# 0xSameer/ast

Hardware: AMD Instinct MI355X
Metric: speech frames/s (train step) (higher is better)
Workload: dtype f32 storage / f32 accumulate; batched GEMMs as bf16x3 splits on the bf16 MFMA pipe (every f32 operand value represented EXACTLY by three bf16 terms, f32 exponent range, six term products, each product exact to 2^-26: >= float32 on any data); the encoder recurrences multiply the same way (resident we

## Files before the change

### ast_amd/_lib.py

```python
import ctypes as C
import os

_HERE = os.path.dirname(os.path.abspath(__file__))
LIB_PATH = os.environ.get("ASTK_LIB_PATH") or os.path.join(_HERE, "libastk.so")

TEST_LIB_PATH = os.path.join(_HERE, "libastk_test.so")

MAX_CNN = 4
MAX_RNN = 8
MAX_ATTN = 4
ENCODE_ROWS_MAX = 32
PREC_DEFAULT, PREC_FP16X2, PREC_BF16X3, PREC_F32 = 0, 1, 2, 3
OPERANDS_DEFAULT, OPERANDS_F32, OPERANDS_FP16 = 0, 1, 2
OPERANDS_BY_NAME = {None: OPERANDS_DEFAULT, "default": OPERANDS_DEFAULT, "f32": OPERANDS_F32, "fp16": OPERANDS_FP16}
PREC_BY_NAME = {None: PREC_DEFAULT, "default": PREC_DEFAULT, "fp16x2": PREC_FP16X2, "bf16x3": PREC_BF16X3, "f32": PREC_F32}

c_float_p = C.POINTER(C.c_float)
c_int_p = C.POINTER(C.c_int32)
c_double_p = C.POINTER(C.c_double)


class _Sized:

    def __init__(self, *a, **k):
# ... 178 lines not shown
    "astk_sample_topk_workspace_bytes": (_SZ, [C.POINTER(DecoderDesc), _I]),
    "astk_sample_decode_topk": (C.c_int, [C.POINTER(DecoderDesc), C.POINTER(DecoderParams), _VP, _VP, _VP, _I, _I, _I, _VP, _F, _I, _F, _VP,
                                          _VP, _VP, _VP, _VP, _VP, _SZ, _VP, _VP]),
    "astk_gumbel_rows": (C.c_int, [_VP, _I, _I, _I, _VP, _VP]),
    "astk_sample_row_key": (_U64, [_U64, _U64]),
    "astk_forced_workspace_bytes": (_SZ, [C.POINTER(DecoderDesc), _I, _I]),
    "astk_forced_score": (C.c_int, [C.POINTER(DecoderDesc), C.POINTER(DecoderParams), _VP, _VP, _VP, _VP, _I, _VP, _VP, _VP, _VP, _VP, _VP, _SZ,
                                    _VP]),
    "astk_greedy_decode_rows": (C.c_int, [C.POINTER(DecoderDesc), C.POINTER(DecoderParams), _VP, _VP, _VP, _I, _I, _I, _VP, _VP, _VP, _VP,
                                          _SZ, _VP, _VP]),
    "astk_greedy_decode_scored_rows": (C.c_int, [C.POINTER(DecoderDesc), C.POINTER(DecoderParams), _VP, _VP, _VP, _I, _I, _I, _VP, _I, _VP,
                                                 _VP, _VP, _VP, _VP, _VP, _VP, _SZ, _VP, _VP]),
    "astk_sample_decode_rows": (C.c_int, [C.POINTER(DecoderDesc), C.POINTER(DecoderParams), _VP, _VP, _VP, _I, _I, _I, _VP, _F, _VP, _VP, _VP,
                                          _VP, _VP, _SZ, _VP, _VP]),
    "astk_forced_score_rows": (C.c_int, [C.POINTER(DecoderDesc), C.POINTER(DecoderParams), _VP, _VP, _VP, _VP, _I, _VP, _VP, _VP, _VP, _VP,
                                         _VP, _SZ, _VP, _VP]),
    "astk_beam_workspace_bytes": (_SZ, [C.POINTER(BeamDesc), C.POINTER(DecoderDesc)]),
    "astk_beam_step": (C.c_int, [C.POINTER(BeamDesc), C.POINTER(DecoderDesc), C.POINTER(DecoderParams), _VP, C.POINTER(BeamState), _I, _VP,
                                 _SZ, _VP]),
    "astk_beam_select": (C.c_int, [C.POINTER(BeamDesc), _I, _I, _I, _VP, _VP, _L, _VP, _VP, _VP, C.POINTER(BeamState), _I, _VP]),
    "astk_beam_decode_workspace_bytes": (_SZ, [C.POINTER(DecoderDesc), _I, _I, _I, _I]),
    "astk_beam_decode": (C.c_int, [C.POINTER(DecoderDesc), C.POINTER(DecoderParams), _VP, _VP, _VP, _VP, _I, _I, _I, _I, _I, _VP, _VP, _VP, _VP,
                                   _VP, _VP, _VP, _VP, _VP, _VP, _SZ, _VP]),
    "astk_attn_step_fwd_rows": (C.c_int, [_I, _I, _I, _VP, _VP, _VP, _VP, _VP, _VP, _VP, _SZ, _VP]),
    "astk_spin": (C.c_int, [C.c_uint, _VP, _VP]),
    "astk_softmax_ce_fwd": (C.c_int, [_I, _I, _L, _VP, _VP, _L, _VP, _F, _VP, _VP, _VP]),
    "astk_softmax_ce_fwd_ex": (C.c_int, [_I, _I, _L, _VP, _VP, _L, _VP, _F, _F, _VP, _VP, _VP]),
    "astk_grad_sqnorm": (C.c_int, [_VP, _VP, _F, _SZ, _VP, _VP]),
    "astk_decay_clip_amsgrad_step": (C.c_int, [_VP, _VP, _VP, _VP, _VP, _SZ, _F, _F, _VP, _F, C.c_double, C.c_double, _F, _I, _VP]),
    "astk_decay_clip_sgd_step": (C.c_int, [_VP, _VP, _SZ, _F, _F, _VP, _F, _VP]),
    "astk_grad_sqnorm_scaled": (C.c_int, [_VP, _VP, _F, _F, _SZ, _VP, _VP]),
    "astk_decay_clip_amsgrad_step_scaled": (C.c_int, [_VP, _VP, _VP, _VP, _VP, _SZ, _F, _F, _F, _VP, _F, C.c_double, C.c_double, _F, _I, _VP]),
    "astk_decay_clip_sgd_step_scaled": (C.c_int, [_VP, _VP, _SZ, _F, _F, _F, _VP, _F, _VP]),
    "astk_decay_clip_noise": (C.c_int, [_VP, _VP, _SZ, _F, _F, _F, _VP, _F, _U64, _U64, _VP]),
    "astk_fill_dropout_mask": (C.c_int, [_VP, _SZ, _F, _U64, _U64, _VP]),
    "astk_fill_normal": (C.c_int, [_VP, _SZ, _F, _F, _U64, _U64, _VP]),
    "astk_fill_random": (C.c_int, [C.POINTER(RandSeg), _I, _VP]),
    "astk_fill_random_ex": (C.c_int, [C.POINTER(RandSeg), _I, C.POINTER(C.c_int32), _I, _VP, _VP]),
    "astk_scale_f32": (C.c_int, [_VP, _SZ, _F, _VP]),
    "astk_add_f32": (C.c_int, [_VP, _VP, _SZ, _VP]),
    "astk_bridge_states": (C.c_int, [_VP, _VP, _VP, _VP, C.c_int, C.c_int, C.c_int, C.c_int, C.c_int, C.c_int, _VP]),
    "astk_colsum_add_f32": (C.c_int, [_VP, _VP, _L, _I, _I, _VP]),
    "astk_zero_frames": (C.c_int, [_VP, _I, _I, _I, _VP, C.c_double, _U64, _U64, _VP]),
    "astk_zero_frames_draws": (C.c_int, [_I, _I, _VP, C.c_double, _U64, _U64, _VP, _I, _VP, _VP]),
    "astk_persist_status_snapshot": (C.c_int, [_VP, _VP]),
    "astk_persist_status_merge": (C.c_int, [_VP, _VP]),
    "astk_persist_status": (C.c_int, [C.POINTER(C.c_uint), _I]),
    "astk_device_cu_count": (C.c_int, []),
    "astk_lstm_stack_path": (C.c_int, [C.POINTER(LstmStackDesc)]),
    "astk_lstm_stack_free_cus": (C.c_int, [C.POINTER(LstmStackDesc)]),
    "astk_lstm_stack_side_plan": (C.c_int, [C.POINTER(LstmStackDesc), C.POINTER(C.c_int), C.POINTER(C.c_int), C.POINTER(C.c_int)]),
    "astk_decoder_path": (C.c_int, [C.POINTER(DecoderDesc)]),
    "astk_prof_begin": (C.c_int, []),
    "astk_prof_end": (C.c_int, [C.POINTER(C.c_double)]),
}

TEST_HOOK_SIGNATURES = {
    "astk_debug_set_amax_generation": (C.c_int, [C.c_uint]),
    "astk_conv_debug_preact": (C.c_int, [C.POINTER(CnnDesc), _VP, _SZ, _I, _VP, _VP]),
    "astk_conv_debug_kill_units": (C.c_int, [_VP, _I]),
    "astk_debug_gemm_group": (C.c_int, [_I, _I, c_int_p, c_int_p, c_int_p, C.POINTER(C.c_void_p), C.POINTER(C.c_void_p), C.POINTER(C.c_void_p), _I, _I, _VP]),
    "astk_debug_gemm_plan": (C.c_int, [_I, _I] + [c_int_p] * 7 + [_I] * 6 + [C.c_char_p, _SZ]),
    "astk_debug_rowgemm": (C.c_int, [C.POINTER(DebugRowGemmArgs), c_int_p, _VP]),
    "astk_debug_lstm_cell_fwd": (C.c_int, [C.POINTER(DebugCellFwdArgs), _I, c_int_p, _VP]),
    "astk_debug_lstm_cell_bwd": (C.c_int, [C.POINTER(DebugCellBwdArgs), _I, c_int_p, _VP]),
}

_lib = None
_test_lib = None


class AstkError(RuntimeError):
    pass


def load():
    global _lib
    if _lib is not None:
        return _lib
    try:
        import torch
    except ImportError:
        pass
    if not os.path.exists(LIB_PATH):
        raise AstkError(f"{LIB_PATH} not found: build it with `python -c 'import __graft_entry__ as g; g.build()'` "
                        "(there is no CPU or PyTorch fallback for the compute path)")
    lib = C.CDLL(LIB_PATH)
    _bind(lib, SIGNATURES)
    _lib = lib
    return lib


def _bind(lib, sigs):
    for name, (res, args) in sigs.items():
        fn = getattr(lib, name)
# ... 64 lines not shown
```

### ast_amd/csrc/common.h

```cpp
#pragma once
#include <hip/hip_runtime.h>
#include <stdint.h>
#include <stddef.h>
#include <stdio.h>
#include <string.h>
#include "../../include/astk.h"

namespace astk {

void set_error(const char* fmt, ...);

enum ProfCat { PROF_ATTN_FWD = 0, PROF_ATTN_BWD = 1, PROF_GEMM = 2, PROF_CELL = 3, PROF_DEC_FWD = 4, PROF_DEC_BWD = 5, PROF_NCAT = 6 };
bool prof_enabled();
float* prof_tick_buffer(int which);
void prof_start(int cat, hipStream_t s, double work);
void prof_stop(int cat, hipStream_t s);
void prof_add_bytes(int cat, double bytes);
struct ProfScope {
  int cat; hipStream_t s; bool on;
  ProfScope(int c, hipStream_t st, double work = 0.0) : cat(c), s(st), on(prof_enabled()) { if (on) prof_start(cat, s, work); }
  ~ProfScope() { if (on) prof_stop(cat, s); }
};

#define ASTK_CHECK(cond, ...)            \
// ... 3 lines not shown
      return -1;                         \
    }                                    \
  } while (0)

#define ASTK_CHECK_DESC(d, type)                                                                                                        \
  ASTK_CHECK((d) != nullptr && (d)->struct_size == sizeof(type),                                                                         \
             #type ": null descriptor or struct_size %zu != %zu (zero-initialise the struct, set struct_size = sizeof(" #type "), astk.h)", \
             (d) ? (size_t)(d)->struct_size : (size_t)0, sizeof(type))

#define ASTK_HIP(expr)                                                               \
  do {                                                                               \
    hipError_t e_ = (expr);                                                          \
    if (e_ != hipSuccess) {                                                          \
      astk::set_error("%s failed: %s (%s:%d)", #expr, hipGetErrorString(e_), __FILE__, __LINE__); \
      return -2;                                                                     \
    }                                                                                \
  } while (0)

#define ASTK_LAUNCH_CHECK()                                                          \
  do {                                                                               \
    hipError_t e_ = hipGetLastError();                                               \
    if (e_ != hipSuccess) {                                                          \
      astk::set_error("kernel launch failed: %s (%s:%d)", hipGetErrorString(e_), __FILE__, __LINE__); \
      return -3;                                                                     \
    }                                                                                \
  } while (0)

#define ASTK_TRY(expr)        \
  do {                        \
    int r_ = (expr);          \
    if (r_ != 0) return r_;   \
  } while (0)

enum PersistBit { PERSIST_ENC_FWD = 1, PERSIST_ENC_BWD = 2, PERSIST_DEC_FWD = 4, PERSIST_DEC_BWD = 8 };
struct AbortCtl {
  unsigned* word;
  unsigned* status;
  unsigned limit;
  unsigned bit;
};
AbortCtl abort_ctl(unsigned* word, unsigned bit);
int device_cu_count();
enum TuneKey {
  TUNE_GEMM_TILE, TUNE_GEMM_T256_ABOVE, TUNE_GEMM_GRID, TUNE_GEMM_HYBRID, TUNE_GEMM_CHUNK, TUNE_GEMM_CHUNK_DIV, TUNE_GEMM_LOG, TUNE_GEMM_TICKET,
  TUNE_GEMM_DETERMINISTIC, TUNE_GEMM_FORWARD_PAIRS,
  TUNE_CONV_DIRECT0, TUNE_CONV_SEQ_FWD, TUNE_CONV_SEQ_BWD, TUNE_CONV_SEQ_STATS_BLOCKS, TUNE_CONV_SEQ_APPLY_BLOCKS,
  TUNE_DEC_PERSIST, TUNE_DEC_B6_SPLIT, TUNE_DEC_B6_FUSED, TUNE_DEC_WIDE,
  TUNE_LSTM_PERSIST, TUNE_LSTM_HOIST, TUNE_LSTM_X3, TUNE_LSTM_X4, TUNE_LSTM_ROWS32, TUNE_LSTM_OVERLAP_CHUNK, TUNE_LSTM_SIDE_FWD, TUNE_LSTM_SIDE_BWD, TUNE_LSTM_DUO_SIDE,
  TUNE_ROW_LONGK, TUNE_PERSIST_SPIN_LIMIT, TUNE_COLREDUCE_BLOCKS,
  TUNE_COUNT
};
double tune(TuneKey k);
inline bool tune_on(TuneKey k) { return tune(k) != 0.0; }
__device__ __forceinline__ bool abort_seen(const AbortCtl& ab) {
  return __hip_atomic_load(ab.word, __ATOMIC_RELAXED, __HIP_MEMORY_SCOPE_AGENT) != 0;
}
__device__ __forceinline__ void abort_raise(const AbortCtl& ab) {
  __hip_atomic_store(ab.word, 1u, __ATOMIC_RELAXED, __HIP_MEMORY_SCOPE_AGENT);
  __hip_atomic_fetch_or(ab.status, ab.bit, __ATOMIC_RELAXED, __HIP_MEMORY_SCOPE_AGENT);
}

constexpr int AMAX_SLOT_WORDS = 16;
constexpr int AMAX_PSLOT_STRIDE = 16;
constexpr int AMAX_PSLOT_WORDS = AMAX_SLOT_WORDS * AMAX_PSLOT_STRIDE;
static inline unsigned long long* amax_pslot_handle(unsigned long long* p) { return p ? (unsigned long long*)((uintptr_t)p | 1u) : nullptr; }
static inline __host__ __device__ unsigned long long* amax_shard(const unsigned long long* handle, int i) {
  unsigned long long* base = (unsigned long long*)((uintptr_t)handle & ~(uintptr_t)1);
  return base + (i & (AMAX_SLOT_WORDS - 1)) * (((uintptr_t)handle & 1u) ? AMAX_PSLOT_STRIDE : 1);
}

typedef float f32x4 __attribute__((ext_vector_type(4)));
typedef float f32x16 __attribute__((ext_vector_type(16)));
__device__ __forceinline__ float wave_sum(float v) {
#pragma unroll
  for (int o = 32; o > 0; o >>= 1) v += __shfl_xor(v, o);
  return v;
}

#if defined(__HIPCC__)
typedef _Float16 h16x2 __attribute__((ext_vector_type(2)));
typedef _Float16 h16x8 __attribute__((ext_vector_type(8)));
typedef unsigned u32q __attribute__((ext_vector_type(4)));
// ... 440 lines not shown
```

### ast_amd/csrc/util.hip

```cpp
#include "common.h"
#include <algorithm>
#include <stdarg.h>
#include <vector>
#include <atomic>
#include <mutex>

namespace astk {

static thread_local char g_err[512] = "";

void set_error(const char* fmt, ...) {
  va_list ap;
  va_start(ap, fmt);
  vsnprintf(g_err, sizeof(g_err), fmt, ap);
  va_end(ap);
}
const char* last_error() { return g_err; }

struct ProfState {
  bool on = false;
  std::vector<hipEvent_t> ev[PROF_NCAT];
  double work[PROF_NCAT] = {0, 0, 0, 0, 0, 0};
  double bytes[PROF_NCAT] = {0, 0, 0, 0, 0, 0};
};
static ProfState g_prof;
static float* g_tick = nullptr;
float* prof_tick_buffer(int which) { return (g_prof.on && g_tick) ? g_tick + 512 * which : nullptr; }
bool prof_enabled() { return g_prof.on; }
void prof_add_bytes(int cat, double bytes) { if (g_prof.on) g_prof.bytes[cat] += bytes; }
void prof_start(int cat, hipStream_t s, double work) {
  hipEvent_t e;
  if (hipEventCreate(&e) != hipSuccess) return;
  (void)hipEventRecord(e, s);
// ... 34 lines not shown
struct TuneEntry { TuneKey key; const char* name; double def; };
static constexpr TuneEntry g_tune_table[TUNE_COUNT] = {
    {TUNE_GEMM_TILE, "gemm.tile", 0},
    {TUNE_GEMM_T256_ABOVE, "gemm.t256_above", 2e10},
    {TUNE_GEMM_GRID, "gemm.grid", -1},
    {TUNE_GEMM_HYBRID, "gemm.hybrid", 1},
    {TUNE_GEMM_CHUNK, "gemm.chunk", 1},
    {TUNE_GEMM_CHUNK_DIV, "gemm.chunk_div", 4},
    {TUNE_GEMM_LOG, "gemm.log", 0},
    {TUNE_GEMM_TICKET, "gemm.ticket", 1},
    {TUNE_GEMM_DETERMINISTIC, "gemm.deterministic", 0},
    {TUNE_GEMM_FORWARD_PAIRS, "gemm.forward_pairs", 1},
    {TUNE_CONV_DIRECT0, "conv.direct0", 1},
    {TUNE_CONV_SEQ_FWD, "conv.seq_fwd", 1},
    {TUNE_CONV_SEQ_BWD, "conv.seq_bwd", 1},
    {TUNE_CONV_SEQ_STATS_BLOCKS, "conv.seq_stats_blocks", 1024},
    {TUNE_CONV_SEQ_APPLY_BLOCKS, "conv.seq_apply_blocks", 1024},
    {TUNE_DEC_PERSIST, "dec.persist", 1},
    {TUNE_DEC_B6_SPLIT, "dec.b6_split", 1},
    {TUNE_DEC_B6_FUSED, "dec.b6_fused", 1},
    {TUNE_DEC_WIDE, "dec.wide", 1},
    {TUNE_LSTM_PERSIST, "lstm.persist", 1},
    {TUNE_LSTM_HOIST, "lstm.hoist", 1},
    {TUNE_LSTM_X3, "lstm.x3", 1},
    {TUNE_LSTM_X4, "lstm.x4", 1},
    {TUNE_LSTM_ROWS32, "lstm.rows32", -1},
    {TUNE_LSTM_OVERLAP_CHUNK, "lstm.overlap_chunk", 0},
    {TUNE_LSTM_SIDE_FWD, "lstm.side_fwd", 1},
    {TUNE_LSTM_SIDE_BWD, "lstm.side_bwd", 0},
    {TUNE_LSTM_DUO_SIDE, "lstm.duo_side", 0},
    {TUNE_ROW_LONGK, "row.longk", 2048},
    {TUNE_PERSIST_SPIN_LIMIT, "persist.spin_limit", 0},
    {TUNE_COLREDUCE_BLOCKS, "colreduce.blocks", 256},
};
constexpr bool tune_table_in_order() {
  for (int i = 0; i < TUNE_COUNT; ++i)
    if (g_tune_table[i].key != i) return false;
  return true;
}
static_assert(tune_table_in_order(), "g_tune_table rows must follow enum TuneKey");
static std::atomic<double> g_tune[TUNE_COUNT];
static std::atomic<int> g_tune_init{0};
static void tune_init() {
  if (g_tune_init.load(std::memory_order_acquire)) return;
  static std::mutex mu;
  std::lock_guard<std::mutex> lock(mu);
  if (g_tune_init.load()) return;
  for (int i = 0; i < TUNE_COUNT; ++i) g_tune[i].store(g_tune_table[i].def);
  g_tune_init.store(1, std::memory_order_release);
}
double tune(TuneKey k) { tune_init(); return g_tune[k].load(std::memory_order_relaxed); }
static int tune_find(const char* key) {
  if (!key) return -1;
  for (int i = 0; i < TUNE_COUNT; ++i)
    if (!strcmp(key, g_tune_table[i].name)) return i;
  return -1;
}

int device_cu_count() {
  int dev = 0;
  if (hipGetDevice(&dev) != hipSuccess || dev < 0 || dev >= 16) return 0;
  if (g_cu_count[dev] == 0) {
    int n = 0;
    if (hipDeviceGetAttribute(&n, hipDeviceAttributeMultiprocessorCount, dev) != hipSuccess) return 0;
    g_cu_count[dev] = n;
  }
// ... 256 lines not shown
    const float gi = decayed_grad(gi_raw, gsc, l2, pi) * gs;
    mi += omb1 * (gi - mi);
    vi += omb2 * (gi * gi - vi);
    vh = amsgrad ? fmaxf(vh, vi) : vi;
    pi = pi - lr_t * mi / (sqrtf(vh) + eps);
  };
  const size_t stride = (size_t)gridDim.x * blockDim.x, tid = blockIdx.x * (size_t)blockDim.x + threadIdx.x;
  size_t done = 0;
  if (((((uintptr_t)p) | ((uintptr_t)g) | ((uintptr_t)m) | ((uintptr_t)v) | ((uintptr_t)(amsgrad ? vhat : p))) & 15) == 0) {
    const size_t n4 = n / 4;
    float4* p4 = reinterpret_cast<float4*>(p);
    const float4* g4 = reinterpret_cast<const float4*>(g);
    float4 *m4 = reinterpret_cast<float4*>(m), *v4 = reinterpret_cast<float4*>(v), *h4 = reinterpret_cast<float4*>(vhat);
    for (size_t i = tid; i < n4; i += stride) {
      float4 P = p4[i], M = m4[i], V = v4[i], H = amsgrad ? h4[i] : make_float4(0.f, 0.f, 0.f, 0.f);
      const float4 G = g4[i];
      one(P.x, G.x, M.x, V.x, H.x); one(P.y, G.y, M.y, V.y, H.y); one(P.z, G.z, M.z, V.z, H.z); one(P.w, G.w, M.w, V.w, H.w);
      m4[i] = M; v4[i] = V;
      if (amsgrad) h4[i] = H;
      p4[i] = P;
    }
    done = n4 * 4;
  }
  for (size_t i = done + tid; i < n; i += stride) {
    float pi = p[i], mi = m[i], vi = v[i], vh = amsgrad ? vhat[i] : 0.f;
    one(pi, g[i], mi, vi, vh);
    m[i] = mi;
    v[i] = vi;
    if (amsgrad) vhat[i] = vh;
    p[i] = pi;
  }
}

__global__ void k_decay_clip_noise(float* g, const float* p, size_t n, float gsc, float l2, float clip, const double* sqnorm, float sigma,
                                   uint64_t seed, uint64_t offset) {
  const float norm = (float)sqrt(*sqnorm);
  const float rate = clip / norm;
  const float gs = rate < 1.f ? rate : 1.f;
  const size_t pairs = (n + 1) / 2;
  for (size_t i = blockIdx.x * (size_t)blockDim.x + threadIdx.x; i < pairs; i += (size_t)gridDim.x * blockDim.x) {
    const uint64_t b = mix64(seed ^ mix64(offset + i));
    const float u1 = u01(b), u2 = u01(mix64(b));
    const float r = sqrtf(-2.f * logf(u1));
    float sn, cs;
    sincosf(6.2831853071795864f * u2, &sn, &cs);
    g[2 * i] = decayed_grad(g[2 * i], gsc, l2, p[2 * i]) * gs + sigma * r * cs;
    if (2 * i + 1 < n) g[2 * i + 1] = decayed_grad(g[2 * i + 1], gsc, l2, p[2 * i + 1]) * gs + sigma * r * sn;
  }
}

__global__ void k_sgd(float* p, const float* g, size_t n, float gsc, float l2, float clip, const double* sqnorm, float lr, const unsigned* status) {
  if (status && *status != 0u) return;
  const float norm = (float)sqrt(*sqnorm);
  const float rate = clip / norm;
  const float gs = rate < 1.f ? rate : 1.f;
  for (size_t i = blockIdx.x * (size_t)blockDim.x + threadIdx.x; i < n; i += (size_t)gridDim.x * blockDim.x)
    p[i] -= lr * decayed_grad(g[i], gsc, l2, p[i]) * gs;
}

inline unsigned grid_for(size_t n, int per = 256) {
  size_t b = (n + per - 1) / per;
  if (b < 1) b = 1;
  if (b > 2048) b = 2048;
  return (unsigned)b;
}

// ... 149 lines not shown
extern "C" {

int astk_version(void) { return ASTK_VERSION; }
const char* astk_last_error(void) { return astk::last_error(); }

int astk_grad_sqnorm(const float* g, const float* p, float l2, size_t n, double* sqnorm, void* stream) {
  return astk_grad_sqnorm_scaled(g, p, 1.f, l2, n, sqnorm, stream);
}
int astk_grad_sqnorm_scaled(const float* g, const float* p, float grad_scale, float l2, size_t n, double* sqnorm, void* stream) {
  hipStream_t s = (hipStream_t)stream;
  ASTK_CHECK(g && p && sqnorm, "grad_sqnorm: null pointer");
  ASTK_CHECK(aligned16(g) && aligned16(p), "grad_sqnorm: buffers must be 16-byte aligned");
  hipLaunchKernelGGL(k_sqnorm, dim3(std::min(SQNORM_BLOCKS, grid_for(n / 4 + 1))), dim3(256), 0, s, g, p, grad_scale, l2, n, sqnorm);
  ASTK_LAUNCH_CHECK();
  return 0;
}

int astk_decay_clip_amsgrad_step(float* p, const float* g, float* m, float* v, float* vhat, size_t n, float l2, float clip,
                                 const double* sqnorm, float lr_t, double beta1, double beta2, float eps, int amsgrad,
                                 void* stream) {
  return astk_decay_clip_amsgrad_step_scaled(p, g, m, v, vhat, n, 1.f, l2, clip, sqnorm, lr_t, beta1, beta2, eps, amsgrad, stream);
}
int astk_decay_clip_amsgrad_step_scaled(float* p, const float* g, float* m, float* v, float* vhat, size_t n, float grad_scale, float l2,
                                        float clip, const double* sqnorm, float lr_t, double beta1, double beta2, float eps, int amsgrad,
                                        void* stream) {
  ASTK_CHECK(p && g && m && v && sqnorm && (vhat || !amsgrad), "amsgrad_step: null pointer");
  if (n == 0) return 0;
  const float omb1 = (float)(1.0 - beta1), omb2 = (float)(1.0 - beta2);
  hipLaunchKernelGGL(k_amsgrad, dim3(grid_for(n)), dim3(256), 0, (hipStream_t)stream, p, g, m, v, vhat, n, grad_scale, l2, clip, sqnorm,
                     lr_t, omb1, omb2, eps, amsgrad, (const unsigned*)persist_status_ptr());
  ASTK_LAUNCH_CHECK();
  return 0;
}

int astk_decay_clip_sgd_step(float* p, const float* g, size_t n, float l2, float clip, const double* sqnorm, float lr,
                             void* stream) {
  return astk_decay_clip_sgd_step_scaled(p, g, n, 1.f, l2, clip, sqnorm, lr, stream);
}
int astk_decay_clip_sgd_step_scaled(float* p, const float* g, size_t n, float grad_scale, float l2, float clip, const double* sqnorm,
                                    float lr, void* stream) {
  ASTK_CHECK(p && g && sqnorm, "sgd_step: null pointer");
  if (n == 0) return 0;
  hipLaunchKernelGGL(k_sgd, dim3(grid_for(n)), dim3(256), 0, (hipStream_t)stream, p, g, n, grad_scale, l2, clip, sqnorm, lr,
                     (const unsigned*)persist_status_ptr());
  ASTK_LAUNCH_CHECK();
  return 0;
}

int astk_decay_clip_noise(float* g, const float* p, size_t n, float grad_scale, float l2, float clip, const double* sqnorm, float sigma,
                          uint64_t seed, uint64_t offset, void* stream) {
  ASTK_CHECK(g && p && sqnorm && sigma >= 0.f, "decay_clip_noise: bad arguments");
  if (n == 0) return 0;
  hipLaunchKernelGGL(k_decay_clip_noise, dim3(grid_for((n + 1) / 2)), dim3(256), 0, (hipStream_t)stream, g, p, n, grad_scale, l2, clip, sqnorm,
                     sigma, seed, offset);
  ASTK_LAUNCH_CHECK();
  return 0;
}

int astk_fill_dropout_mask(float* out, size_t n, float ratio, uint64_t seed, uint64_t offset, void* stream) {
  ASTK_CHECK(out && ratio >= 0.f && ratio < 1.f, "fill_dropout_mask: bad arguments");
  if (n == 0) return 0;
  hipLaunchKernelGGL(k_dropout_mask, dim3(grid_for(n)), dim3(256), 0, (hipStream_t)stream, out, n, ratio, 1.f / (1.f - ratio),
                     seed, offset);
  ASTK_LAUNCH_CHECK();
  return 0;
}
// ... 201 lines not shown
```

### ast_amd/optimizers.py

```python
import ctypes as C
import math

import torch

from . import _lib
from ._lib import check


class WeightDecay:
    def __init__(self, rate):
        self.rate = rate


class GradientClipping:
    def __init__(self, threshold):
        self.threshold = threshold


class GradientNoise:

    def __init__(self, eta, seed=0x6E015E):
        self.eta = float(eta)
        self.seed = seed
        self.offset = 0
# ... 13 lines not shown
        return self

    def add_hook(self, hook):
        if isinstance(hook, WeightDecay) and any(isinstance(h, (GradientClipping, GradientNoise)) for h in self.hooks):
            raise NotImplementedError("the fused update implements the reference's order WeightDecay -> GradientClipping -> GradientNoise")
        if isinstance(hook, GradientClipping) and any(isinstance(h, GradientNoise) for h in self.hooks):
            raise NotImplementedError("the fused update implements the reference's order WeightDecay -> GradientClipping -> GradientNoise")
        self.hooks.append(hook)

    def _apply_noise(self, lib, a, l2, clip, s):
        noise = [h for h in self.hooks if isinstance(h, GradientNoise)]
        if not noise:
            return l2, clip, self.grad_scale
        h = noise[0]
        sigma = math.sqrt(h.eta / (1.0 + (self.t - 1)) ** 0.55)
        frozen = getattr(self.target, "_frozen", set())
        for name, shp in a.shapes.items():
            if name.split("/")[0] in frozen:
                continue
            off, n = a.offsets[name], 1
            for d in shp:
                n *= int(d)
            check(lib.astk_decay_clip_noise(C.c_void_p(a.grad.data_ptr() + 4 * off), C.c_void_p(a.data.data_ptr() + 4 * off), n, self.grad_scale,
                                            l2, clip, C.c_void_p(self.sqnorm.data_ptr()), sigma, h.seed, h.offset, s))
            h.offset += (n + 1) // 2
        return 0.0, 3.0e38, 1.0

    def _hook_values(self):
        l2 = sum(h.rate for h in self.hooks if isinstance(h, WeightDecay))
        clips = [h.threshold for h in self.hooks if isinstance(h, GradientClipping)]
        clip = float(clips[0]) if clips else float("inf")
        return float(l2), clip

    def _prepare(self):
        m = self.target
        lib = _lib.load()
        a = m.arena
        if self.sqnorm is None:
            self.sqnorm = torch.zeros(1, dtype=torch.float64, device=a.device)
        self.grad_scale = 1.0
        if self.grad_sync is not None:
            r = self.grad_sync(a)
            if isinstance(r, float):
                self.grad_scale = r
        l2, clip = self._hook_values()
        s = C.c_void_p(torch.cuda.current_stream(a.device).cuda_stream)
        check(lib.astk_grad_sqnorm_scaled(C.c_void_p(a.grad.data_ptr()), C.c_void_p(a.data.data_ptr()), self.grad_scale, l2, a.size,
                                          C.c_void_p(self.sqnorm.data_ptr()), s))
        if clip == float("inf"):
            clip = 3.0e38
        return lib, a, l2, clip, s

    @property
    def last_grad_norm(self):
        return math.sqrt(float(self.sqnorm.item()))


class Adam(_Optimizer):
    def __init__(self, alpha=0.001, beta1=0.9, beta2=0.999, eps=1e-8, amsgrad=False):
        super().__init__()
        self.alpha, self.beta1, self.beta2, self.eps, self.amsgrad = alpha, beta1, beta2, eps, amsgrad
        self.m = self.v = self.vhat = None

    def update(self):
        lib, a, l2, clip, s = self._prepare()
        if self.m is None:
            self.m = torch.zeros_like(a.data)
            self.v = torch.zeros_like(a.data)
            self.vhat = torch.zeros_like(a.data)
        self.t += 1
        lr_t = self.alpha * math.sqrt(1.0 - self.beta2 ** self.t) / (1.0 - self.beta1 ** self.t)
        l2, clip, gscale = self._apply_noise(lib, a, l2, clip, s)
        for off, n in self.target.enabled_ranges():
            def p(t):
                return C.c_void_p(t.data_ptr() + 4 * off)
            check(lib.astk_decay_clip_amsgrad_step_scaled(p(a.data), p(a.grad), p(self.m), p(self.v), p(self.vhat), n, gscale, l2,
                                                          clip, C.c_void_p(self.sqnorm.data_ptr()), lr_t, self.beta1, self.beta2,
                                                          self.eps, 1 if self.amsgrad else 0, s))


class SGD(_Optimizer):
    def __init__(self, lr=0.01):
        super().__init__()
        self.lr = lr

    def update(self):
        lib, a, l2, clip, s = self._prepare()
        self.t += 1
        l2, clip, gscale = self._apply_noise(lib, a, l2, clip, s)
        for off, n in self.target.enabled_ranges():
            check(lib.astk_decay_clip_sgd_step_scaled(C.c_void_p(a.data.data_ptr() + 4 * off), C.c_void_p(a.grad.data_ptr() + 4 * off), n,
                                                      gscale, l2, clip, C.c_void_p(self.sqnorm.data_ptr()), self.lr, s))
```

### include/astk.h

```cpp
#ifndef ASTK_H
#define ASTK_H
#include <stddef.h>
#include <stdint.h>

#ifdef __cplusplus
extern "C" {
#endif

#define ASTK_VERSION 108
#define ASTK_MAX_CNN_LAYERS 4
#define ASTK_MAX_RNN_LAYERS 8
#define ASTK_MAX_ATTN 4

int astk_version(void);
const char* astk_last_error(void);

enum { ASTK_PREC_DEFAULT = 0, ASTK_PREC_FP16X2 = 1, ASTK_PREC_BF16X3 = 2, ASTK_PREC_F32 = 3 };
enum { ASTK_OPERANDS_DEFAULT = 0, ASTK_OPERANDS_F32 = 1, ASTK_OPERANDS_FP16 = 2 };

int astk_gemm_f32(int layout, int M, int N, int K,
                  const float* A, long lda, const float* B, long ldb, float* C, long ldc,
                  const float* bias, int mode, int ksplit, int batch, long sA, long sB, long sC, void* stream);
int astk_gemm_f32_ex(int layout, int M, int N, int K,
                     const float* A, long lda, const float* B, long ldb, float* C, long ldc,
// ... 269 lines not shown
                     int32_t* hist, int32_t* slot_status, double* score, float* c_fin, float* h_fin, float* ht_fin, float* alpha,
                     void* ws, size_t ws_bytes, void* stream);

int astk_attn_step_fwd_rows(int R, int T, int H, const float* enc, const int32_t* row_utt, const int32_t* row_len, const float* q,
                            float* alpha, float* cv, void* ws, size_t ws_bytes, void* stream);

int astk_layernorm_fwd(int rows, int n, const float* x, long ldx, const float* gamma, const float* beta, float eps, float* y, long ldy,
                       void* stream);
int astk_layernorm_bwd(int rows, int n, const float* x, long ldx, const float* gamma, float eps, const float* dy, long lddy, float* dx,
                       long lddx, float* dgamma, float* dbeta, void* stream);
int astk_step_bn_relu_fwd(int T, int B, int C, const float* z, const float* gamma, const float* beta, float* avg_mean, float* avg_var,
                          float eps, float decay, int train, float* out, float* stats, void* stream);
int astk_step_bn_relu_bwd(int T, int B, int C, const float* z, const float* stats, const float* gamma, float eps, const float* out,
                          const float* d_out, float* dz, float* dgamma, float* dbeta, void* stream);

int astk_softmax_ce_fwd(int B, int V, long ld, float* logits_inout, const int32_t* targets, long t_stride,
                        const float* class_weight, float inv_count, float* loss_rows, int32_t* argmax, void* stream);
int astk_softmax_ce_fwd_ex(int B, int V, long ld, float* logits_inout, const int32_t* targets, long t_stride,
                           const float* class_weight, float inv_count, float label_smoothing, float* loss_rows, int32_t* argmax,
                           void* stream);

int astk_grad_sqnorm(const float* g, const float* p, float l2, size_t n, double* sqnorm, void* stream);
int astk_decay_clip_amsgrad_step(float* p, const float* g, float* m, float* v, float* vhat, size_t n,
                                 float l2, float clip, const double* sqnorm, float lr_t, double beta1, double beta2,
                                 float eps, int amsgrad, void* stream);
int astk_decay_clip_sgd_step(float* p, const float* g, size_t n, float l2, float clip, const double* sqnorm,
                             float lr, void* stream);
int astk_grad_sqnorm_scaled(const float* g, const float* p, float grad_scale, float l2, size_t n, double* sqnorm, void* stream);
int astk_decay_clip_amsgrad_step_scaled(float* p, const float* g, float* m, float* v, float* vhat, size_t n, float grad_scale,
                                        float l2, float clip, const double* sqnorm, float lr_t, double beta1, double beta2,
                                        float eps, int amsgrad, void* stream);
int astk_decay_clip_sgd_step_scaled(float* p, const float* g, size_t n, float grad_scale, float l2, float clip,
                                    const double* sqnorm, float lr, void* stream);

int astk_fill_dropout_mask(float* out, size_t n, float ratio, uint64_t seed, uint64_t offset, void* stream);
int astk_decay_clip_noise(float* g, const float* p, size_t n, float grad_scale, float l2, float clip, const double* sqnorm, float sigma,
                          uint64_t seed, uint64_t offset, void* stream);
int astk_fill_normal(float* out, size_t n, float mean, float sigma, uint64_t seed, uint64_t offset, void* stream);
#define ASTK_RAND_SEG_MAX 8
#define ASTK_RAND_DROPOUT 0
#define ASTK_RAND_NORMAL 1
typedef struct {
  float* out;
  size_t n;
  int kind;
  float a, b;
  uint64_t seed, offset;
} astk_rand_seg;
int astk_fill_random(const astk_rand_seg* segs, int n_segs, void* stream);
#define ASTK_RAND_WORDS_MAX 256
int astk_fill_random_ex(const astk_rand_seg* segs, int n_segs, const int32_t* words, int n_words, int32_t* words_dst, void* stream);
int astk_scale_f32(float* x, size_t n, float s, void* stream);
int astk_add_f32(float* dst, const float* src, size_t n, void* stream);
int astk_colsum_add_f32(float* dst, const float* src, long lds, int rows, int cols, void* stream);
int astk_bridge_states(float* dec_c, float* dec_h, float* enc_c, float* enc_h, int nd, int nl_enc, int n, int B, int h, int to_decoder,
                       void* stream);
int astk_zero_frames(float* X, int B, int T, int D, const int32_t* lengths, double rate, uint64_t seed, uint64_t offset, void* stream);
int astk_zero_frames_draws(int B, int T, const int32_t* lengths, double rate, uint64_t seed, uint64_t offset, int32_t* idx, int max_draws,
                           int32_t* counts, void* stream);
int astk_spin(unsigned usec, unsigned* flag, void* stream);

int astk_persist_status_snapshot(float* dst, void* stream);
int astk_persist_status_merge(const float* summed, void* stream);
int astk_lstm_stack_path(const astk_lstm_stack_desc* d);
int astk_lstm_stack_free_cus(const astk_lstm_stack_desc* d);
int astk_lstm_stack_side_plan(const astk_lstm_stack_desc* d, int* fwd_head_steps, int* fwd_chunks, int* bwd_chunks);
// ... 81 lines not shown
```

Before: 4.668 million.

## Fuse gradient norm and AMSGrad step into one grid-synchronised resident kernel

Result: no change. 4.678 million, median of 3 (+0.2%).

```diff
diff --git a/ast_amd/_lib.py b/ast_amd/_lib.py
--- a/ast_amd/_lib.py
+++ b/ast_amd/_lib.py
@@ -234,6 +234,7 @@
     "astk_grad_sqnorm_scaled": (C.c_int, [_VP, _VP, _F, _F, _SZ, _VP, _VP]),
     "astk_decay_clip_amsgrad_step_scaled": (C.c_int, [_VP, _VP, _VP, _VP, _VP, _SZ, _F, _F, _F, _VP, _F, C.c_double, C.c_double, _F, _I, _VP]),
     "astk_decay_clip_sgd_step_scaled": (C.c_int, [_VP, _VP, _SZ, _F, _F, _F, _VP, _F, _VP]),
+    "astk_decay_clip_amsgrad_step_fused": (C.c_int, [_VP, _VP, _VP, _VP, _VP, _SZ, _F, _F, _F, _VP, _F, C.c_double, C.c_double, _F, _I, _VP]),
     "astk_decay_clip_noise": (C.c_int, [_VP, _VP, _SZ, _F, _F, _F, _VP, _F, _U64, _U64, _VP]),
     "astk_fill_dropout_mask": (C.c_int, [_VP, _SZ, _F, _U64, _U64, _VP]),
     "astk_fill_normal": (C.c_int, [_VP, _SZ, _F, _F, _U64, _U64, _VP]),
@@ -263,6 +264,7 @@
     "astk_conv_debug_kill_units": (C.c_int, [_VP, _I]),
     "astk_debug_gemm_group": (C.c_int, [_I, _I, c_int_p, c_int_p, c_int_p, C.POINTER(C.c_void_p), C.POINTER(C.c_void_p), C.POINTER(C.c_void_p), _I, _I, _VP]),
     "astk_debug_gemm_plan": (C.c_int, [_I, _I] + [c_int_p] * 7 + [_I] * 6 + [C.c_char_p, _SZ]),
+    "astk_debug_resident_partition": (C.c_int, [C.c_longlong, _I, _I, C.POINTER(C.c_longlong), c_int_p]),
     "astk_debug_rowgemm": (C.c_int, [C.POINTER(DebugRowGemmArgs), c_int_p, _VP]),
     "astk_debug_lstm_cell_fwd": (C.c_int, [C.POINTER(DebugCellFwdArgs), _I, c_int_p, _VP]),
     "astk_debug_lstm_cell_bwd": (C.c_int, [C.POINTER(DebugCellBwdArgs), _I, c_int_p, _VP]),
diff --git a/ast_amd/csrc/common.h b/ast_amd/csrc/common.h
--- a/ast_amd/csrc/common.h
+++ b/ast_amd/csrc/common.h
@@ -59,7 +59,7 @@
     if (r_ != 0) return r_;   \
   } while (0)
 
-enum PersistBit { PERSIST_ENC_FWD = 1, PERSIST_ENC_BWD = 2, PERSIST_DEC_FWD = 4, PERSIST_DEC_BWD = 8 };
+enum PersistBit { PERSIST_ENC_FWD = 1, PERSIST_ENC_BWD = 2, PERSIST_DEC_FWD = 4, PERSIST_DEC_BWD = 8, PERSIST_RESIDENT = 32 };
 struct AbortCtl {
   unsigned* word;
   unsigned* status;
@@ -74,7 +74,7 @@
   TUNE_CONV_DIRECT0, TUNE_CONV_SEQ_FWD, TUNE_CONV_SEQ_BWD, TUNE_CONV_SEQ_STATS_BLOCKS, TUNE_CONV_SEQ_APPLY_BLOCKS,
   TUNE_DEC_PERSIST, TUNE_DEC_B6_SPLIT, TUNE_DEC_B6_FUSED, TUNE_DEC_WIDE,
   TUNE_LSTM_PERSIST, TUNE_LSTM_HOIST, TUNE_LSTM_X3, TUNE_LSTM_X4, TUNE_LSTM_ROWS32, TUNE_LSTM_OVERLAP_CHUNK, TUNE_LSTM_SIDE_FWD, TUNE_LSTM_SIDE_BWD, TUNE_LSTM_DUO_SIDE,
-  TUNE_ROW_LONGK, TUNE_PERSIST_SPIN_LIMIT, TUNE_COLREDUCE_BLOCKS,
+  TUNE_ROW_LONGK, TUNE_PERSIST_SPIN_LIMIT, TUNE_COLREDUCE_BLOCKS, TUNE_OPT_RESIDENT,
   TUNE_COUNT
 };
 double tune(TuneKey k);
diff --git a/ast_amd/csrc/resident_pass.h b/ast_amd/csrc/resident_pass.h
--- /dev/null
+++ b/ast_amd/csrc/resident_pass.h
@@ -0,0 +1,104 @@
+#pragma once
+#include "common.h"
+
+namespace astk {
+
+constexpr int RP_THREADS = 512;
+constexpr int RP_MAX_GRID = 512;
+constexpr int RP_MAX_R = 16;
+
+struct ResidentPart {
+  int grid;
+  int R;
+  long long units;
+  long long resident;
+  long long streamed;
+};
+constexpr int resident_R_choices[] = {1, 2, 4, 8, RP_MAX_R};
+inline ResidentPart resident_partition(long long units, int capacity, int cap) {
+  ResidentPart p;
+  if (capacity > RP_MAX_GRID) capacity = RP_MAX_GRID;
+  if (capacity < 1) capacity = 1;
+  if (units < 0) units = 0;
+  const long long wgs = (units + RP_THREADS - 1) / RP_THREADS;
+  p.grid = (int)(wgs < 1 ? 1 : wgs > capacity ? capacity : wgs);
+  const long long per_thread = (units + (long long)p.grid * RP_THREADS - 1) / ((long long)p.grid * RP_THREADS);
+  if (cap > RP_MAX_R) cap = RP_MAX_R;
+  p.R = 0;
+  for (int r : resident_R_choices) {
+    if (r > cap) break;
+    p.R = r;
+    if (r >= per_thread) break;
+  }
+  p.units = units;
+  const long long room = (long long)p.grid * RP_THREADS * p.R;
+  p.resident = units < room ? units : room;
+  p.streamed = units - p.resident;
+  return p;
+}
+inline void resident_owner(const ResidentPart& p, long long u, int* wg, int* thread, int* slot) {
+  const long long G = (long long)p.grid * RP_THREADS;
+  const long long gt = (u < p.resident ? u : u - p.resident) % G;
+  *wg = (int)(gt / RP_THREADS);
+  *thread = (int)(gt % RP_THREADS);
+  *slot = u < p.resident ? (int)(u / G) : -1;
+}
+
+#if defined(__HIPCC__)
+struct RpMeet {
+  unsigned* ctr;
+  double* part;
+};
+template <typename K>
+int resident_capacity(K kernel) {
+  int per_cu = 0;
+  if (hipOccupancyMaxActiveBlocksPerMultiprocessor(&per_cu, kernel, RP_THREADS, 0) != hipSuccess) { (void)hipGetLastError(); return 0; }
+  const int cus = device_cu_count();
+  if (per_cu < 1 || cus < 1) return 0;
+  return cus * per_cu;
+}
+#endif
+
+}
+
+#if defined(__HIPCC__)
+#include "handoff.h"
+namespace astk {
+namespace {
+
+__device__ __forceinline__ double rp_block_sum(double s, double* red) {
+#pragma unroll
+  for (int o = 32; o > 0; o >>= 1) s += __shfl_xor(s, o);
+  __syncthreads();
+  if ((threadIdx.x & 63) == 0) red[threadIdx.x >> 6] = s;
+  __syncthreads();
+  double t = 0.0;
+#pragma unroll
+  for (int w = 0; w < RP_THREADS / 64; ++w) t += red[w];
+  return t;
+}
+__device__ __forceinline__ bool rp_arrive(const RpMeet& mt, double partial, const AbortCtl& ab, int* s_flag) {
+  if (threadIdx.x == 0) {
+    __hip_atomic_store(&mt.part[blockIdx.x], partial, __ATOMIC_RELAXED, __HIP_MEMORY_SCOPE_AGENT);
+    asm volatile("s_waitcnt vmcnt(0)" ::: "memory");
+    __hip_atomic_fetch_add(mt.ctr, 1u, __ATOMIC_RELAXED, __HIP_MEMORY_SCOPE_AGENT);
+    *s_flag = (wait_ge(mt.ctr, gridDim.x, ab) && !abort_seen(ab)) ? 1 : 0;
+  }
+  __syncthreads();
+  return *s_flag != 0;
+}
+__device__ __forceinline__ double rp_fold(const RpMeet& mt, double* red) {
+  const double v = threadIdx.x < gridDim.x ? __hip_atomic_load(&mt.part[threadIdx.x], __ATOMIC_RELAXED, __HIP_MEMORY_SCOPE_AGENT) : 0.0;
+  return rp_block_sum(v, red);
+}
+__device__ __forceinline__ void rp_leave(const RpMeet& mt) {
+  if (threadIdx.x == 0 && __hip_atomic_fetch_add(mt.ctr + CTRS, 1u, __ATOMIC_RELAXED, __HIP_MEMORY_SCOPE_AGENT) == gridDim.x - 1) {
+    __hip_atomic_store(mt.ctr, 0u, __ATOMIC_RELAXED, __HIP_MEMORY_SCOPE_AGENT);
+    __hip_atomic_store(mt.ctr + CTRS, 0u, __ATOMIC_RELAXED, __HIP_MEMORY_SCOPE_AGENT);
+    __hip_atomic_store(mt.ctr + 2 * CTRS, 0u, __ATOMIC_RELAXED, __HIP_MEMORY_SCOPE_AGENT);
+  }
+}
+
+}
+}
+#endif
diff --git a/ast_amd/csrc/util.hip b/ast_amd/csrc/util.hip
--- a/ast_amd/csrc/util.hip
+++ b/ast_amd/csrc/util.hip
@@ -1,4 +1,5 @@
 #include "common.h"
+#include "resident_pass.h"
 #include <algorithm>
 #include <stdarg.h>
 #include <vector>
@@ -99,6 +100,7 @@
     {TUNE_ROW_LONGK, "row.longk", 2048},
     {TUNE_PERSIST_SPIN_LIMIT, "persist.spin_limit", 0},
     {TUNE_COLREDUCE_BLOCKS, "colreduce.blocks", 256},
+    {TUNE_OPT_RESIDENT, "opt.resident", RP_MAX_R},
 };
 constexpr bool tune_table_in_order() {
   for (int i = 0; i < TUNE_COUNT; ++i)
@@ -421,6 +423,129 @@
   }
 }
 
+__device__ unsigned g_rp_opt_ctr[3 * CTRS];
+__device__ double g_rp_opt_part[RP_MAX_GRID];
+struct AdamArgs { float gsc, l2, clip, lr_t, omb1, omb2, eps; int amsgrad; };
+__device__ __forceinline__ double sq_term(float a, float b, float gsc, float l2) {
+  const float x = decayed_grad(a, gsc, l2, b);
+  return (double)x * x;
+}
+__device__ __forceinline__ double sq_term(const float4& a, const float4& b, float gsc, float l2) {
+  const float x = decayed_grad(a.x, gsc, l2, b.x), y = decayed_grad(a.y, gsc, l2, b.y), z = decayed_grad(a.z, gsc, l2, b.z), w = decayed_grad(a.w, gsc, l2, b.w);
+  return (double)(x * x + y * y) + (double)(z * z + w * w);
+}
+__device__ __forceinline__ void adam_one(float& pi, float gi_raw, float& mi, float& vi, float& vh, const AdamArgs& a, float gs) {
+  const float gi = decayed_grad(gi_raw, a.gsc, a.l2, pi) * gs;
+  mi += a.omb1 * (gi - mi);
+  vi += a.omb2 * (gi * gi - vi);
+  vh = a.amsgrad ? fmaxf(vh, vi) : vi;
+  pi = pi - a.lr_t * mi / (sqrtf(vh) + a.eps);
+}
+__device__ __forceinline__ void adam_one(float4& P, const float4& G, float4& M, float4& V, float4& H, const AdamArgs& a, float gs) {
+  adam_one(P.x, G.x, M.x, V.x, H.x, a, gs); adam_one(P.y, G.y, M.y, V.y, H.y, a, gs);
+  adam_one(P.z, G.z, M.z, V.z, H.z, a, gs); adam_one(P.w, G.w, M.w, V.w, H.w, a, gs);
+}
+__device__ __forceinline__ void rp_zero(float& x) { x = 0.f; }
+__device__ __forceinline__ void rp_zero(float4& x) { x = make_float4(0.f, 0.f, 0.f, 0.f); }
+template <typename U>
+__device__ __forceinline__ void adam_unit(U* p, U* m, U* v, U* vhat, size_t i, U P, const U& G, const AdamArgs& a, float gs) {
+  U M = m[i], V = v[i], H;
+  if (a.amsgrad) H = vhat[i]; else rp_zero(H);
+  adam_one(P, G, M, V, H, a, gs);
+  m[i] = M; v[i] = V;
+  if (a.amsgrad) vhat[i] = H;
+  p[i] = P;
+}
+template <int R, typename U>
+__global__ __launch_bounds__(RP_THREADS) void k_amsgrad_resident(float* p, const float* g, float* m, float* v, float* vhat, size_t n, size_t resident,
+                                                                 AdamArgs a, double* sqnorm, RpMeet mt, AbortCtl ab) {
+  __shared__ double red[RP_THREADS / 64];
+  __shared__ int s_flag;
+  constexpr size_t W = sizeof(U) / sizeof(float);
+  const size_t units = n / W;
+  const size_t G = (size_t)gridDim.x * RP_THREADS, gt = blockIdx.x * (size_t)RP_THREADS + threadIdx.x;
+  U* pu = reinterpret_cast<U*>(p);
+  const U* gu = reinterpret_cast<const U*>(g);
+  U gq[R], pq[R];
+#pragma unroll
+  for (int j = 0; j < R; ++j) {
+    const size_t i = gt + j * G;
+    if (i < resident) { gq[j] = gu[i]; pq[j] = pu[i]; } else { rp_zero(gq[j]); rp_zero(pq[j]); }
+  }
+  double s = 0.0;
+#pragma unroll
+  for (int j = 0; j < R; ++j) s += sq_term(gq[j], pq[j], a.gsc, a.l2);
+  for (size_t i = resident + gt; i < units; i += G) s += sq_term(gu[i], pu[i], a.gsc, a.l2);
+  if (blockIdx.x == 0 && units * W + threadIdx.x < n) s += sq_term(g[units * W + threadIdx.x], p[units * W + threadIdx.x], a.gsc, a.l2);
+  const double part = rp_block_sum(s, red);
+  if (rp_arrive(mt, part, ab, &s_flag)) {
+    const double total = rp_fold(mt, red);
+    if (blockIdx.x == 0 && threadIdx.x == 0) *sqnorm = total;
+    if (ld_flag(ab.status) == 0u) {
+      const float norm = (float)sqrt(total);
+      const float rate = a.clip / norm;
+      const float gs = rate < 1.f ? rate : 1.f;
+      U *mu = reinterpret_cast<U*>(m), *vu = reinterpret_cast<U*>(v), *hu = reinterpret_cast<U*>(vhat);
+#pragma unroll
+      for (int j = 0; j < R; ++j) {
+        const size_t i = gt + j * G;
+        if (i < resident) adam_unit(pu, mu, vu, hu, i, pq[j], gq[j], a, gs);
+      }
+      for (size_t i = resident + gt; i < units; i += G) adam_unit(pu, mu, vu, hu, i, pu[i], gu[i], a, gs);
+      if (blockIdx.x == 0 && units * W + threadIdx.x < n) {
+        const size_t i = units * W + threadIdx.x;
+        adam_unit(p, m, v, vhat, i, p[i], g[i], a, gs);
+      }
+    }
+  }
+  rp_leave(mt);
+}
+typedef void (*OptResidentKernel)(float*, const float*, float*, float*, float*, size_t, size_t, AdamArgs, double*, RpMeet, AbortCtl);
+struct OptResidentPlan { OptResidentKernel launch; ResidentPart part; };
+template <typename U>
+OptResidentKernel opt_resident_kernel(int R) {
+  switch (R) {
+    case 1: return k_amsgrad_resident<1, U>;
+    case 2: return k_amsgrad_resident<2, U>;
+    case 4: return k_amsgrad_resident<4, U>;
+    case 8: return k_amsgrad_resident<8, U>;
+    case RP_MAX_R: return k_amsgrad_resident<RP_MAX_R, U>;
+  }
+  return nullptr;
+}
+int opt_resident_plan(const float* p, const float* g, const float* m, const float* v, const float* h, size_t n, OptResidentPlan* out) {
+  out->launch = nullptr;
+  const int cap = (int)tune(TUNE_OPT_RESIDENT);
+  const int cus = device_cu_count();
+  if (cap <= 0 || cus < 1) return 0;
+  const bool vec = ((((uintptr_t)p) | ((uintptr_t)g) | ((uintptr_t)m) | ((uintptr_t)v) | ((uintptr_t)h)) & 15) == 0;
+  out->part = resident_partition((long long)(vec ? n / 4 : n), cus, cap);
+  OptResidentKernel k = vec ? opt_resident_kernel<float4>(out->part.R) : opt_resident_kernel<float>(out->part.R);
+  ASTK_CHECK(k, "amsgrad_step_fused: no kernel for %d resident units", out->part.R);
+  static std::atomic<int> capacity[2][RP_MAX_R + 1];
+  int c = capacity[vec][out->part.R].load();
+  if (c == 0) {
+    c = resident_capacity(k);
+    capacity[vec][out->part.R].store(c > 0 ? c : -1);
+  }
+  if (c >= cus) out->launch = k;
+  return 0;
+}
+static unsigned* rp_opt_ctr_ptr() {
+  static unsigned* ptr[16] = {nullptr};
+  int dev = 0;
+  if (hipGetDevice(&dev) != hipSuccess || dev < 0 || dev >= 16) dev = 0;
+  if (!ptr[dev] && hipGetSymbolAddress((void**)&ptr[dev], HIP_SYMBOL(g_rp_opt_ctr)) != hipSuccess) return nullptr;
+  return ptr[dev];
+}
+static double* rp_opt_part_ptr() {
+  static double* ptr[16] = {nullptr};
+  int dev = 0;
+  if (hipGetDevice(&dev) != hipSuccess || dev < 0 || dev >= 16) dev = 0;
+  if (!ptr[dev] && hipGetSymbolAddress((void**)&ptr[dev], HIP_SYMBOL(g_rp_opt_part)) != hipSuccess) return nullptr;
+  return ptr[dev];
+}
+
 __global__ void k_decay_clip_noise(float* g, const float* p, size_t n, float gsc, float l2, float clip, const double* sqnorm, float sigma,
                                    uint64_t seed, uint64_t offset) {
   const float norm = (float)sqrt(*sqnorm);
@@ -636,6 +761,44 @@
   ASTK_LAUNCH_CHECK();
   return 0;
 }
+
+int astk_decay_clip_amsgrad_step_fused(float* p, const float* g, float* m, float* v, float* vhat, size_t n, float grad_scale, float l2,
+                                       float clip, double* sqnorm, float lr_t, double beta1, double beta2, float eps, int amsgrad,
+                                       void* stream) {
+  ASTK_CHECK(p && g && m && v && sqnorm && (vhat || !amsgrad), "amsgrad_step_fused: null pointer");
+  ASTK_CHECK(n > 0, "amsgrad_step_fused: empty range (the norm is a sum over it)");
+  OptResidentPlan plan;
+  ASTK_TRY(opt_resident_plan(p, g, m, v, amsgrad ? vhat : p, n, &plan));
+  if (!plan.launch) {
+    ASTK_TRY(astk_grad_sqnorm_scaled(g, p, grad_scale, l2, n, sqnorm, stream));
+    return astk_decay_clip_amsgrad_step_scaled(p, g, m, v, vhat, n, grad_scale, l2, clip, sqnorm, lr_t, beta1, beta2, eps, amsgrad, stream);
+  }
+  unsigned* ctr = rp_opt_ctr_ptr();
+  double* part = rp_opt_part_ptr();
+  ASTK_CHECK(ctr && part && persist_status_ptr(), "amsgrad_step_fused: no meeting place");
+  const AdamArgs a = {grad_scale, l2, clip, lr_t, (float)(1.0 - beta1), (float)(1.0 - beta2), eps, amsgrad};
+  const RpMeet mt = {ctr, part};
+  const AbortCtl ab = abort_ctl(ctr + 2 * CTRS, PERSIST_RESIDENT);
+  hipLaunchKernelGGL(plan.launch, dim3(plan.part.grid), dim3(RP_THREADS), 0, (hipStream_t)stream, p, g, m, v, vhat, n, (size_t)plan.part.resident,
+                     a, sqnorm, mt, ab);
+  ASTK_LAUNCH_CHECK();
+  return 0;
+}
+
+#ifdef ASTK_TEST_HOOKS
+int astk_debug_resident_partition(long long units, int capacity, int cap, long long* part, int32_t* owner) {
+  ASTK_CHECK(part && units >= 0 && capacity >= 1 && cap >= 1, "debug_resident_partition: bad arguments");
+  const ResidentPart P = resident_partition(units, capacity, cap);
+  part[0] = P.grid; part[1] = P.R; part[2] = P.units; part[3] = P.resident; part[4] = P.streamed;
+  if (owner)
+    for (long long u = 0; u < units; ++u) {
+      int w, t, j;
+      resident_owner(P, u, &w, &t, &j);
+      owner[3 * u] = w; owner[3 * u + 1] = t; owner[3 * u + 2] = j;
+    }
+  return RP_THREADS;
+}
+#endif
 
 int astk_decay_clip_sgd_step(float* p, const float* g, size_t n, float l2, float clip, const double* sqnorm, float lr,
                              void* stream) {
diff --git a/ast_amd/optimizers.py b/ast_amd/optimizers.py
--- a/ast_amd/optimizers.py
+++ b/ast_amd/optimizers.py
@@ -69,7 +69,7 @@
         clip = float(clips[0]) if clips else float("inf")
         return float(l2), clip
 
-    def _prepare(self):
+    def _prepare(self, norm=True):
         m = self.target
         lib = _lib.load()
         a = m.arena
@@ -82,8 +82,9 @@
                 self.grad_scale = r
         l2, clip = self._hook_values()
         s = C.c_void_p(torch.cuda.current_stream(a.device).cuda_stream)
-        check(lib.astk_grad_sqnorm_scaled(C.c_void_p(a.grad.data_ptr()), C.c_void_p(a.data.data_ptr()), self.grad_scale, l2, a.size,
-                                          C.c_void_p(self.sqnorm.data_ptr()), s))
+        if norm:
+            check(lib.astk_grad_sqnorm_scaled(C.c_void_p(a.grad.data_ptr()), C.c_void_p(a.data.data_ptr()), self.grad_scale, l2, a.size,
+                                              C.c_void_p(self.sqnorm.data_ptr()), s))
         if clip == float("inf"):
             clip = 3.0e38
         return lib, a, l2, clip, s
@@ -100,15 +101,23 @@
         self.m = self.v = self.vhat = None
 
     def update(self):
-        lib, a, l2, clip, s = self._prepare()
+        ranges = self.target.enabled_ranges()
+        one_launch = ranges == [(0, self.target.arena.size)] and not any(isinstance(h, GradientNoise) for h in self.hooks)
+        lib, a, l2, clip, s = self._prepare(norm=not one_launch)
         if self.m is None:
             self.m = torch.zeros_like(a.data)
             self.v = torch.zeros_like(a.data)
             self.vhat = torch.zeros_like(a.data)
         self.t += 1
         lr_t = self.alpha * math.sqrt(1.0 - self.beta2 ** self.t) / (1.0 - self.beta1 ** self.t)
+        if one_launch:
+            def q(t):
+                return C.c_void_p(t.data_ptr())
+            check(lib.astk_decay_clip_amsgrad_step_fused(q(a.data), q(a.grad), q(self.m), q(self.v), q(self.vhat), a.size, self.grad_scale, l2, clip,
+                                                         q(self.sqnorm), lr_t, self.beta1, self.beta2, self.eps, 1 if self.amsgrad else 0, s))
+            return
         l2, clip, gscale = self._apply_noise(lib, a, l2, clip, s)
-        for off, n in self.target.enabled_ranges():
+        for off, n in ranges:
             def p(t):
                 return C.c_void_p(t.data_ptr() + 4 * off)
             check(lib.astk_decay_clip_amsgrad_step_scaled(p(a.data), p(a.grad), p(self.m), p(self.v), p(self.vhat), n, gscale, l2,
diff --git a/include/astk.h b/include/astk.h
--- a/include/astk.h
+++ b/include/astk.h
@@ -325,6 +325,12 @@
                                         float eps, int amsgrad, void* stream);
 int astk_decay_clip_sgd_step_scaled(float* p, const float* g, size_t n, float grad_scale, float l2, float clip,
                                     const double* sqnorm, float lr, void* stream);
+int astk_decay_clip_amsgrad_step_fused(float* p, const float* g, float* m, float* v, float* vhat, size_t n, float grad_scale,
+                                       float l2, float clip, double* sqnorm, float lr_t, double beta1, double beta2,
+                                       float eps, int amsgrad, void* stream);
+#ifdef ASTK_TEST_HOOKS
+int astk_debug_resident_partition(long long units, int capacity, int cap, long long* part, int32_t* owner);
+#endif
 
 int astk_fill_dropout_mask(float* out, size_t n, float ratio, uint64_t seed, uint64_t offset, void* stream);
 int astk_decay_clip_noise(float* g, const float* p, size_t n, float grad_scale, float l2, float clip, const double* sqnorm, float sigma,
```
